# MLAB-project/radio-observer

Measured on AMD Instinct MI355X. Metric: FFT rows/sec (spectra/sec), N=32768 75% overlap, incl. per-row bolid scan, higher is better.
Workload: dtype f32; 1 GPU; C3/C4: synthetic IQ 48 kHz, FFT bins=32768, overlap=24576 (75%), Nuttall window, waterfall magnitude rows + BolidRecorder scan; input=float32 I/Q resident in HBM, output=float32 rows in HBM, parallelism=time-chunk per GPU

## Files before the change

radio-observer_amd/csrc/ro_k32_lds.h:

```cpp
#pragma once

#include "ro_fft_device.h"
#include "ro_device_util.h"

namespace ro {
namespace k32 {

constexpr int N = 32768, T = 1024, H = 16;
constexpr int RQ = 1026;
constexpr int IMAGE_BYTES = 32 * RQ * 4;
constexpr int LDS_BYTES = IMAGE_BYTES + 1024;
constexpr int HB = 61692;
constexpr int XB = 3972;
static_assert(HB % 4 == 0 && 15 * 256 + HB <= 65535 && 31 * 4 * RQ - HB <= 65535 && 16 * 4 * RQ - HB >= 0,
              "rows 16..31: M0 / offset split");
static_assert(XB % 4 == 0 && 15 * 4 * RQ + XB <= 65535 && 4 * 16 * RQ + 15 * 256 - XB <= 65535 && 4 * 16 * RQ - XB >= 0,
              "exchange 1, odd slots: M0 / offset split");

template <int Q>
__device__ __forceinline__ void x1_write_pair(unsigned ma, unsigned mb, float s_q, float s_q1, float s_q16, float s_q17)
{
    static_assert(Q % 2 == 0 && Q < 16, "slot algebra");
    constexpr int E = 256 * (Q >> 1), O = 4 * 16 * RQ - XB + 256 * (Q >> 1);
    addtid_write4<E, E + 2048, O, O + 2048>(ma, mb, s_q, s_q16, s_q1, s_q17);
}
template <typename F> __device__ __forceinline__ void x1_write_plane(unsigned ma, unsigned mb, F f)
{
    constexpr int O = 4 * 16 * RQ - XB;
    addtid_write8<0, 256, 512, 768, 1024, 1280, 1536, 1792>(ma, f(0), f(2), f(4), f(6), f(8), f(10), f(12), f(14));
    addtid_write8<2048, 2304, 2560, 2816, 3072, 3328, 3584, 3840>(ma, f(16), f(18), f(20), f(22), f(24), f(26), f(28), f(30));
    addtid_write8<O, O + 256, O + 512, O + 768, O + 1024, O + 1280, O + 1536, O + 1792>(mb, f(1), f(3), f(5), f(7), f(9), f(11),
                                                                                        f(13), f(15));
    addtid_write8<O + 2048, O + 2304, O + 2560, O + 2816, O + 3072, O + 3328, O + 3584, O + 3840>(
        mb, f(17), f(19), f(21), f(23), f(25), f(27), f(29), f(31));
}
template <int QA, int QB, int QC, int QD>
__device__ __forceinline__ void own_write4(unsigned mc, unsigned md, float sa, float sb, float sc, float sd)
{
    static_assert(QA < 16 && QB < 16 && QC >= 16 && QD >= 16 && QC < 32 && QD < 32, "row algebra");
    constexpr int R = 4 * RQ;
    addtid_write4<R * QA, R * QB, R * QC - HB, R * QD - HB>(mc, md, sa, sb, sc, sd);
}
template <typename F> __device__ __forceinline__ void own_write_plane(unsigned mc, unsigned md, F f)
{
    constexpr int R = 4 * RQ;
    addtid_write8<0 * R, 1 * R, 2 * R, 3 * R, 4 * R, 5 * R, 6 * R, 7 * R>(mc, f(0), f(1), f(2), f(3), f(4), f(5), f(6), f(7));
    addtid_write8<8 * R, 9 * R, 10 * R, 11 * R, 12 * R, 13 * R, 14 * R, 15 * R>(mc, f(8), f(9), f(10), f(11), f(12), f(13),
                                                                                  f(14), f(15));
    addtid_write8<16 * R - HB, 17 * R - HB, 18 * R - HB, 19 * R - HB, 20 * R - HB, 21 * R - HB, 22 * R - HB, 23 * R - HB>(
        md, f(16), f(17), f(18), f(19), f(20), f(21), f(22), f(23));
    addtid_write8<24 * R - HB, 25 * R - HB, 26 * R - HB, 27 * R - HB, 28 * R - HB, 29 * R - HB, 30 * R - HB, 31 * R - HB>(
        md, f(24), f(25), f(26), f(27), f(28), f(29), f(30), f(31));
}

typedef const volatile __attribute__((address_space(3))) v2f lds_vpair;

}
}
```

radio-observer_amd/csrc/ro_stft32k.hip:

```cpp
#define RO_TIE_SCHED 1
#include "ro_kernels.h"
#include "ro_fft_device.h"
#include "ro_fft_planar.h"
#include "ro_device_util.h"
#include "ro_k32_lds.h"

#include <mutex>

#if !defined(RO_DIAG) || !defined(RO_STAMPS32K)
#undef RO_STAMPS32K
#define RO_STAMPS32K 0
#endif

namespace ro {
namespace k32 {

constexpr int PIPE_UNITS = 6;
constexpr int WIN_EARLY = 2;

__host__ __device__ constexpr int column(int t)
{
    const int l = t & 63, j = l & 31;
    return (t & ~63) + 2 * ((j >> 1) + 16 * (j & 1)) + (l >> 5);
}

struct ImageRow {
    const float *img;
    __device__ __forceinline__ float operator()(int c) const
    {
        const int k = (c + N / 2) & (N - 1), r = k >> 10, beta = k & 1023;
        const int w = (beta & 31) >> 1, kb = beta & 1, k1 = beta >> 5;
        return img[RQ * r + 64 * w + 2 * ((k1 - 4 * (w >> 1)) & 31) + kb];
    }
};

template <typename F> __device__ __forceinline__ void dit32_levels123(v2f *v, F hook)
{
    const v2f *tok = &v[31];
    dit_level_order<1>(v, tok, std::make_integer_sequence<int, 2>{});
    hook(std::integral_constant<int, 1>{});
    dit_level_order<2>(v, tok, std::make_integer_sequence<int, 4>{});
    hook(std::integral_constant<int, 2>{});
    dit_level_order<3>(v, tok, std::make_integer_sequence<int, 8>{});
    hook(std::integral_constant<int, 3>{});
}

template <int FMT> __global__ __launch_bounds__(T, 1) void stft32k_kernel(StftArgs a)
{
    extern __shared__ __attribute__((aligned(16))) char smem[];
    using S = Sample<FMT>;
    using namespace planar;

    const int64_t per_xcd = (a.rows + 7) / 8;
    const int64_t xcd_first = (int64_t)(blockIdx.x & 7) * per_xcd;
    const int64_t xcd_end = xcd_first + per_xcd < a.rows ? xcd_first + per_xcd : a.rows;
    const int64_t stride = gridDim.x >> 3;
    int64_t row = xcd_first + (blockIdx.x >> 3);
    if (row >= xcd_end) return;

    const int tid = threadIdx.x;
    const int wave = __builtin_amdgcn_readfirstlane(tid >> 6);
    const __amdgpu_buffer_rsrc_t rs_twk = make_rsrc(a.twiddles_k, (3 * 32 + 3 * 1024) * 16);
    const char *iq = reinterpret_cast<const char *>(a.iq);
    const float *lds = reinterpret_cast<const float *>(smem);

    v2f v[32];

    const int po = (column(tid & ~32) + ((tid >> 5) & 1) * H * (N / 32)) * S::BYTES;
    auto row_rsrc = [&](int64_t k, bool valid) {
        return make_rsrc(iq + (a.first_row + k) * (int64_t)a.hop * S::BYTES, valid ? (unsigned)N * S::BYTES : 0u);
    };
    {
        const __amdgpu_buffer_rsrc_t rs = row_rsrc(row, true);
#pragma unroll
        for (int k = 0; k < H; ++k) S::load_pair(rs, po, k * (N / 32) * S::BYTES, v[k], v[H + k]);
    }
    v4f w4[H / 2];
    auto load_window = [&](const __amdgpu_buffer_rsrc_t &rs_win, auto first_c, auto last_c) {
        constexpr int first = decltype(first_c)::value, last = decltype(last_c)::value;
#pragma unroll
        for (int q = first; q < last; ++q) {
            const u32x4 t = __builtin_amdgcn_raw_buffer_load_b128(rs_win, tid * 16, q * T * 16, 0);
            w4[q] = (v4f){__uint_as_float(t.x), __uint_as_float(t.y), __uint_as_float(t.z), __uint_as_float(t.w)};
        }
    };
    using c0 = std::integral_constant<int, 0>;
    using cE = std::integral_constant<int, WIN_EARLY>;
    using cN = std::integral_constant<int, H / 2>;
    auto win_rsrc = [&](bool valid) { return make_rsrc(a.window_k32, valid ? N * 4 : 0); };
    load_window(win_rsrc(true), c0{}, cN{});

    v2f tw1[5], tw2[5];
    auto tw_load = [&](v2f (&t)[5], int k, auto pk_c, auto ns_c) {
        constexpr int PK = decltype(pk_c)::value, NS = decltype(ns_c)::value;
#pragma unroll
        for (int q = 0; q < 3; ++q) {
            const u32x4 u = __builtin_amdgcn_raw_buffer_load_b128(rs_twk, k * 16, (PK + q * NS) * 16, 0);
            t[2 * q] = (v2f){__uint_as_float(u.x), __uint_as_float(u.y)};
            if (q < 2) t[2 * q + 1] = (v2f){__uint_as_float(u.z), __uint_as_float(u.w)};
        }
    };

    [[maybe_unused]] unsigned long long st_acc[16] = {0, 0, 0, 0, 0, 0, 0, 0, 0, 0, 0, 0, 0, 0, 0, 0}, st_prev = 0;
    auto stamp = [&](int k) {
        if constexpr (RO_STAMPS32K) {
            unsigned long long t;
            __builtin_amdgcn_sched_barrier(0);
            asm volatile("s_memtime %0\n\ts_waitcnt lgkmcnt(0)" : "=s"(t)::"memory");
            __builtin_amdgcn_sched_barrier(0);
            if (k >= 0) st_acc[k] += t - st_prev;
            st_prev = t;
        }
    };
    stamp(-1);
    if constexpr (RO_STAMPS32K) st_acc[13] = __builtin_amdgcn_s_memrealtime();

    const float *prev_out = a.rows_out;
    unsigned prev_bytes = 0;
    unsigned touch = 0;
    int rb_base = RQ * (tid >> 8) + 128 * (tid & 7) + 2 * ((((tid & 255) >> 3) - 4 * (tid & 7)) & 31);
    auto store_chunk = [&](int q, const __amdgpu_buffer_rsrc_t &rs) {
        int rb = rb_base;
        asm volatile("" : "+v"(rb));
        lds_vpair *p = (lds_vpair *)(lds + rb + 4 * RQ * q);
        const v2f x01 = p[0], x23 = p[32];
        buf_store_f4(x01.x, x01.y, x23.x, x23.y, rs, tid * 16, ((q * T * 4 + N / 2) & (N - 1)) * 4);
    };

    const unsigned ma = (unsigned)wave * (4u * RQ), mb = ma + (unsigned)XB;
    const unsigned mc = (unsigned)wave * 256u, md = mc + (unsigned)HB;

    for (;;) {
        const __amdgpu_buffer_rsrc_t rs_prev = make_rsrc(prev_out, prev_bytes);
        {
            const v2f gain2 = (v2f){0.0f, a.gain};
            if (a.gain != 0.0f) {
#pragma unroll
                for (int i = 0; i < 32; ++i) v[i] = v[i] + gain2;
            }
#pragma unroll
            for (int k = 0; k < H; ++k) {
                v2f &lo = v[k], &hi = v[H + k];
                const auto rx = __builtin_amdgcn_permlane32_swap(__float_as_uint(lo.x), __float_as_uint(hi.x), false, false);
                const auto ry = __builtin_amdgcn_permlane32_swap(__float_as_uint(lo.y), __float_as_uint(hi.y), false, false);
                lo = (v2f){__uint_as_float(rx[0]), __uint_as_float(ry[0])};
                hi = (v2f){__uint_as_float(rx[1]), __uint_as_float(ry[1])};
            }
        }
        asm volatile("" ::"v"(touch));
#pragma unroll
        for (int i = 0; i < H; ++i) {
            const v4f c4 = w4[i / 2];
            const v2f wi = (i & 1) ? c4.zz : c4.xx, wj = (i & 1) ? c4.ww : c4.yy;
            const v2f t = v[i] * wi;
            const v2f s = __builtin_elementwise_fma(v[H + i], wj, t);
            v[H + i] = __builtin_elementwise_fma(v[H + i], -wj, t);
            v[i] = s;
            if (i & 1) planar::leash();
        }
        const int64_t next = row + stride;
        const bool has_next = next < xcd_end;
        load_window(win_rsrc(true), c0{}, cE{});
        auto touch_next = [&]() {
            const int64_t s0 = (a.first_row + (has_next ? next : row)) * (int64_t)a.hop + (N - a.hop);
            const __amdgpu_buffer_rsrc_t rs_new =
                make_rsrc(iq + s0 * S::BYTES, (has_next && a.prefetch) ? a.hop * S::BYTES : 0);
            touch = __builtin_amdgcn_raw_buffer_load_b32(rs_new, tid * 128, 0, 0);
        };
        stamp(0);

        store_chunk(0, rs_prev);
        store_chunk(1, rs_prev);
        dit32_levels123(v, [&](auto hc) {
            constexpr int h = decltype(hc)::value;
            store_chunk(2 * h, rs_prev);
            store_chunk(2 * h + 1, rs_prev);
        });
        int lane;
        {
            int lt = tid;
            asm volatile("" : "+v"(lt));
            lane = lt & 63;
        }
        {
            const bool odd = lane >= 32;
            const float4 *tk = a.twiddles_k + 2 * wave;
#pragma unroll
            for (int q = 0; q < 3; ++q) {
                v4f e, o;
                asm volatile("s_load_dwordx4 %0, %2, %3\n\t"
                             "s_load_dwordx4 %1, %2, %4\n\t"
                             "s_waitcnt lgkmcnt(0)"
                             : "=&s"(e), "=&s"(o)
                             : "s"(tk), "n"(q * 32 * 16), "n"(q * 32 * 16 + 16)
                             : "memory");
                tw1[2 * q] = (v2f){odd ? o.x : e.x, odd ? o.y : e.y};
                if (q < 2) tw1[2 * q + 1] = (v2f){odd ? o.z : e.z, odd ? o.w : e.w};
            }
        }
        stamp(1);
        wg_sync();
        stamp(2);
        dit32_last(v, [&](auto jc) {
            constexpr int j = decltype(jc)::value;
            x1_write_pair<bitrev<32>(2 * j)>(ma, mb, v[2 * j].x, v[16 + 2 * j].x, v[2 * j + 1].x, v[17 + 2 * j].x);
            return v[17 + 2 * j].y;
        });
        stamp(3);
        v2f R[16], I[16];
        {
            lds_vpair *g1 = (lds_vpair *)(lds + RQ * 16 * (lane >> 5) + 64 * wave + 2 * (lane & 15) + 32 * ((lane >> 4) & 1));
            asm volatile("s_waitcnt lgkmcnt(0)" ::: "memory");
            __builtin_amdgcn_s_barrier();
            asm volatile("" ::: "memory");
#pragma unroll
            for (int i = 0; i < 16; ++i) R[i] = g1[(RQ / 2) * i];
            wg_sync();
            x1_write_plane(ma, mb, [&](int k0) { return v[bitrev<32>(k0)].y; });
            asm volatile("s_waitcnt lgkmcnt(0)" ::: "memory");
            __builtin_amdgcn_s_barrier();
            asm volatile("" ::: "memory");
#pragma unroll
            for (int i = 0; i < 8; ++i) {
                I[i] = g1[(RQ / 2) * i];
                I[i + 8] = g1[(RQ / 2) * (i + 8)];
            }
        }
        stamp(4);
        planar::head<0>(R, I, tw1[4], tw1[3], tw1[2], tw1[1]);
        touch_next();
        int k1p, kbp;
        {
            k1p = ((lane >> 1) + 4 * (wave >> 1)) & 31;
            kbp = lane & 1;
            tw_load(tw2, 2 * wave + kbp + 32 * k1p, std::integral_constant<int, 96>{}, std::integral_constant<int, 1024>{});
        }
        stamp(5);
        planar::last0(R, I, tw1[0], [&](auto jc) {
            constexpr int j = decltype(jc)::value, q = bitrev<32>(2 * j);
            own_write4<q, q + 1, q + 16, q + 17>(mc, md, R[j].x, R[8 + j].x, R[j].y, R[8 + j].y);
        });
        stamp(6);
        v2f R2[16], I2[16];
        {
            lds_vpair *g2 = (lds_vpair *)(lds + RQ * k1p + 64 * wave + 32 * kbp);
            asm volatile("" ::: "memory");
#pragma unroll
            for (int i = 0; i < 16; ++i) R2[i] = g2[(i >> 1) + 8 * (i & 1)];
            asm volatile("" ::: "memory");
            own_write_plane(mc, md, [&](int k1) {
                constexpr int MB = 0;
                const int p = bitrev<32>(k1);
                return hf<MB>(p) ? I[pr<MB>(p)].y : I[pr<MB>(p)].x;
            });
#pragma unroll
            for (int i = 0; i < 16; ++i) I2[i] = g2[(i >> 1) + 8 * (i & 1)];
        }
        stamp(7);
        planar::head<1>(R2, I2, tw2[4], tw2[3], tw2[2], tw2[1]);
        stamp(8);
        {
            const __amdgpu_buffer_rsrc_t rs_next = row_rsrc(has_next ? next : row, has_next);
            v2f pma = {0.f, 0.f}, pmb = {0.f, 0.f};
            planar::last1(R2, I2, tw2[0], [&](auto uc) {
                constexpr int u = decltype(uc)::value;
                auto mag = [](v2f re, v2f im) {
                    const v2f s = __builtin_elementwise_fma(im, im, re * re);
                    return (v2f){__builtin_amdgcn_sqrtf(s.x), __builtin_amdgcn_sqrtf(s.y)};
                };
                const v2f m_a = mag(R2[2 * u], I2[2 * u]), m_b = mag(R2[2 * u + 1], I2[2 * u + 1]);
                if constexpr (u > 0) {
                    constexpr int r = bitrev<8>(u > 0 ? u - 1 : 0);
                    own_write4<r, r + 8, r + 16, r + 24>(mc, md, pma.x, pma.y, pmb.x, pmb.y);
                }
                pma = m_a;
                pmb = m_b;
                if constexpr (u < PIPE_UNITS) {
                    const int pj = after(po, m_b.y);
                    S::load_pair(rs_next, pj, (2 * u) * (N / 32) * S::BYTES, v[2 * u], v[H + 2 * u]);
                    S::load_pair(rs_next, pj, (2 * u + 1) * (N / 32) * S::BYTES, v[2 * u + 1], v[H + 2 * u + 1]);
                }
            });
            asm volatile("s_nop 7\n\ts_nop 7" ::: "memory");
            {
                constexpr int r = bitrev<8>(7);
                own_write4<r, r + 8, r + 16, r + 24>(mc, md, pma.x, pma.y, pmb.x, pmb.y);
            }
            const bool image_work = (a.records != nullptr && wave < 2) || (a.tile_out != nullptr && (wave == 2 || wave == 3));
            auto late_loads = [&]() {
#pragma unroll
                for (int k = 2 * PIPE_UNITS; k < H; ++k)
                    S::load_pair(rs_next, po, k * (N / 32) * S::BYTES, v[k], v[H + k]);
                load_window(win_rsrc(has_next), cE{}, cN{});
            };
            auto image_complete = [&]() {
                stamp(9);
                asm volatile("s_waitcnt lgkmcnt(0)" ::: "memory");
                wg_sync();
                stamp(10);
            };
            if (!image_work) {
                late_loads();
                image_complete();
            } else {
                image_complete();
                {
                    int sl = tid & 63;
                    asm volatile("" : "+v"(sl));
                    const ImageRow img{lds};
                    if (a.records != nullptr && wave < 2) {
                        int low_noise = a.low_noise, noise_width = a.noise_width, low_detect = a.low_detect;
                        int detect_width = a.detect_width, avg_bins = a.avg_bins;
                        asm volatile("" : "+s"(low_noise), "+s"(noise_width), "+s"(low_detect), "+s"(detect_width), "+s"(avg_bins));
                        if (wave == 0) {
                            unsigned *hist = reinterpret_cast<unsigned *>(smem + IMAGE_BYTES);
                            const float nz = noise_width <= 512 ? scan_noise<8>(img, low_noise, noise_width, hist, sl)
                                                                : scan_noise<0>(img, low_noise, noise_width, hist, sl);
                            if (sl == 0) a.records[row].noise = nz;
                        } else {
                            const int pk = scan_peak<8>(img, low_detect, detect_width, sl);
                            const float av = scan_average(img, low_detect + pk - avg_bins / 2, avg_bins, N, sl);
                            if (sl == 0) {
                                a.records[row].peak = pk;
                                a.records[row].average = av;
                            }
                        }
                    }
                    if (a.tile_out != nullptr && (wave == 2 || wave == 3)) {
                        int tile_cols = a.tile_cols, tile_first = a.tile_first;
                        asm volatile("" : "+s"(tile_cols), "+s"(tile_first));
                        const int half = ((tile_cols + 127) >> 7) << 6;
                        const int c0 = wave == 2 ? 0 : half;
                        const int c1 = wave == 2 ? (half < tile_cols ? half : tile_cols) : tile_cols;
                        float *dst = a.tile_out + row * (int64_t)tile_cols;
                        if (a.ln_out == nullptr) {
                            for (int c = c0 + sl; c < c1; c += 64) dst[c] = img(tile_first + c);
                        } else {
                            float *ldst = a.ln_out + row * (int64_t)tile_cols;
                            unsigned kmin = 0xffffffffu, kmax = 0u;
                            for (int c = c0 + sl; c < c1; c += 64) {
                                const float x = img(tile_first + c);
                                const float l = logf(x);
                                dst[c] = x;
                                ldst[c] = l;
                                if (x != 0.f) {
                                    const unsigned key = order_key(l);
                                    kmin = min(kmin, key);
                                    kmax = max(kmax, key);
                                }
                            }
                            kmin = wave_min_u32(kmin);
                            kmax = wave_max_u32(kmax);
                            if (sl == 0) {
                                float *part = a.ln_part + row * 4 + (wave == 2 ? 0 : 2);
                                part[0] = kmin == 0xffffffffu ? __builtin_inff() : key_to_float(kmin);
                                part[1] = kmax == 0u ? -__builtin_inff() : key_to_float(kmax);
                            }
                        }
                    }
                }
                late_loads();
            }
        }
        stamp(11);
        prev_out = a.rows_out + row * a.row_stride;
        prev_bytes = N * 4;
        if constexpr (RO_STAMPS32K) st_acc[15] += 1;
        if (!has_next) break;
        row = next;
    }
    {
        const __amdgpu_buffer_rsrc_t rs_last = make_rsrc(prev_out, prev_bytes);
#pragma unroll
        for (int q = 0; q < 8; ++q) {
            store_chunk(q, rs_last);
            if (q & 1) asm volatile("" ::: "memory");
        }
    }
    if constexpr (RO_STAMPS32K) {
        st_acc[14] = __builtin_amdgcn_s_memrealtime();
        if (a.stamps && (tid & 63) == 0)
            for (int k = 0; k < 16; ++k) a.stamps[(blockIdx.x * 16 + wave) * 16 + k] = st_acc[k];
    }
}

struct DevicePlan32k {
    bool ready = false;
    int cus = 0;
};

template <int FMT> static hipError_t launch_fmt(const StftArgs &a, hipStream_t s)
{
    static std::mutex lock;
    static DevicePlan32k table[64];
    int dev = 0;
    hipError_t e = hipGetDevice(&dev);
    if (e != hipSuccess) return e;
    if (dev < 0 || dev >= 64) return hipErrorInvalidDevice;
    int cus;
    {
        std::lock_guard<std::mutex> g(lock);
        DevicePlan32k &d = table[dev];
        if (!d.ready) {
            const void *fn = reinterpret_cast<const void *>(&stft32k_kernel<FMT>);
            if ((e = hipFuncSetAttribute(fn, hipFuncAttributeMaxDynamicSharedMemorySize, LDS_BYTES)) != hipSuccess) return e;
            if ((e = hipDeviceGetAttribute(&d.cus, hipDeviceAttributeMultiprocessorCount, dev)) != hipSuccess) return e;
            d.ready = true;
        }
        cus = d.cus;
    }
    const int64_t per_xcd = (a.rows + 7) / 8;
    int64_t slots = cus / 8;
    if (a.spare_cus > 0) slots -= a.spare_cus;
    if (slots < 1) slots = 1;
    if (slots > per_xcd) slots = per_xcd;
    StftArgs b = a;
    b.dec = 1;
    b.dec_log2 = 0;
    b.prefetch = slots * (int64_t)a.hop * Sample<FMT>::BYTES <= (2 << 20) ? 1 : 0;
    b.stagger = 0;
    hipLaunchKernelGGL((stft32k_kernel<FMT>), dim3((unsigned)(slots * 8)), dim3(T), LDS_BYTES, s, b);
    return hipGetLastError();
}

}

void stft32k_window_layout(const float *w, float *out)
{
    using namespace k32;
    for (int t = 0; t < T; ++t) {
        const int c = column(t);
        for (int q = 0; q < H / 2; ++q) {
            float *o = out + ((size_t)q * T + t) * 4;
            o[0] = w[c + 1024 * (2 * q)];
            o[1] = w[c + 1024 * (2 * q + 16)];
            o[2] = w[c + 1024 * (2 * q + 1)];
            o[3] = w[c + 1024 * (2 * q + 17)];
        }
    }
}

hipError_t launch_stft32k(int fmt, const StftArgs &a, hipStream_t s)
{
    if (a.rows <= 0) return hipSuccess;
    if (a.spec_out != nullptr || a.big_form || a.window_k32 == nullptr) return hipErrorInvalidValue;
    if (fmt == RO_FMT_F32) return k32::launch_fmt<RO_FMT_F32>(a, s);
    if (fmt == RO_FMT_I16) return k32::launch_fmt<RO_FMT_I16>(a, s);
    return hipErrorInvalidValue;
}

}
```

Before: 17.56 million rows/s.

## Reschedule first LDS exchange with parked young-wave values and split twiddle loads

New measurement: 16.89 million rows/s. 0.962x the previous value.

```diff
diff --git a/radio-observer_amd/csrc/ro_k32_lds.h b/radio-observer_amd/csrc/ro_k32_lds.h
--- a/radio-observer_amd/csrc/ro_k32_lds.h
+++ b/radio-observer_amd/csrc/ro_k32_lds.h
@@ -17,22 +17,28 @@
 static_assert(XB % 4 == 0 && 15 * 4 * RQ + XB <= 65535 && 4 * 16 * RQ + 15 * 256 - XB <= 65535 && 4 * 16 * RQ - XB >= 0,
               "exchange 1, odd slots: M0 / offset split");
 
+__host__ __device__ constexpr int x1_offset(int k0) { return 256 * (k0 >> 1) + (k0 & 1) * (4 * 16 * RQ - XB); }
+__host__ __device__ constexpr int x1_park_offset(int k0) { return x1_offset(k0 - 16); }
+static_assert(x1_park_offset(16) == 0 && x1_park_offset(17) == 4 * 16 * RQ - XB && x1_park_offset(31) == x1_offset(15),
+              "phase 1 parks y of slot k0 in territory (k0 >> 1) - 8");
+static_assert(x1_park_offset(16) >= 0 && x1_park_offset(31) <= 65535 && x1_park_offset(30) + 15 * 4 * RQ + 252 < IMAGE_BYTES &&
+                  x1_park_offset(31) + 15 * 4 * RQ + XB + 252 < IMAGE_BYTES,
+              "exchange 1, parked y values: M0 / offset split, inside the image");
+static_assert(x1_park_offset(30) + 256 <= x1_offset(16), "parked y values stay below territory 8");
+
 template <int Q>
-__device__ __forceinline__ void x1_write_pair(unsigned ma, unsigned mb, float s_q, float s_q1, float s_q16, float s_q17)
+__device__ __forceinline__ void x1_write_young(unsigned ma, unsigned mb, float x_q16, float y_q16, float x_q17, float y_q17)
 {
     static_assert(Q % 2 == 0 && Q < 16, "slot algebra");
-    constexpr int E = 256 * (Q >> 1), O = 4 * 16 * RQ - XB + 256 * (Q >> 1);
-    addtid_write4<E, E + 2048, O, O + 2048>(ma, mb, s_q, s_q16, s_q1, s_q17);
+    addtid_write4<x1_park_offset(Q + 16), x1_offset(Q + 16), x1_park_offset(Q + 17), x1_offset(Q + 17)>(ma, mb, y_q16, x_q16,
+                                                                                                      y_q17, x_q17);
 }
-template <typename F> __device__ __forceinline__ void x1_write_plane(unsigned ma, unsigned mb, F f)
+template <typename F> __device__ __forceinline__ void x1_write_old(unsigned ma, unsigned mb, F f)
 {
-    constexpr int O = 4 * 16 * RQ - XB;
+    constexpr int O = x1_offset(1);
     addtid_write8<0, 256, 512, 768, 1024, 1280, 1536, 1792>(ma, f(0), f(2), f(4), f(6), f(8), f(10), f(12), f(14));
-    addtid_write8<2048, 2304, 2560, 2816, 3072, 3328, 3584, 3840>(ma, f(16), f(18), f(20), f(22), f(24), f(26), f(28), f(30));
     addtid_write8<O, O + 256, O + 512, O + 768, O + 1024, O + 1280, O + 1536, O + 1792>(mb, f(1), f(3), f(5), f(7), f(9), f(11),
                                                                                         f(13), f(15));
-    addtid_write8<O + 2048, O + 2304, O + 2560, O + 2816, O + 3072, O + 3328, O + 3584, O + 3840>(
-        mb, f(17), f(19), f(21), f(23), f(25), f(27), f(29), f(31));
 }
 template <int QA, int QB, int QC, int QD>
 __device__ __forceinline__ void own_write4(unsigned mc, unsigned md, float sa, float sb, float sc, float sd)
diff --git a/radio-observer_amd/csrc/ro_stft32k.hip b/radio-observer_amd/csrc/ro_stft32k.hip
--- a/radio-observer_amd/csrc/ro_stft32k.hip
+++ b/radio-observer_amd/csrc/ro_stft32k.hip
@@ -160,7 +160,6 @@
         }
         const int64_t next = row + stride;
         const bool has_next = next < xcd_end;
-        load_window(win_rsrc(true), c0{}, cE{});
         auto touch_next = [&]() {
             const int64_t s0 = (a.first_row + (has_next ? next : row)) * (int64_t)a.hop + (N - a.hop);
             const __amdgpu_buffer_rsrc_t rs_new =
@@ -182,11 +181,11 @@
             asm volatile("" : "+v"(lt));
             lane = lt & 63;
         }
-        {
+        auto load_tw1 = [&](auto first_c, auto last_c) {
             const bool odd = lane >= 32;
             const float4 *tk = a.twiddles_k + 2 * wave;
 #pragma unroll
-            for (int q = 0; q < 3; ++q) {
+            for (int q = decltype(first_c)::value; q < decltype(last_c)::value; ++q) {
                 v4f e, o;
                 asm volatile("s_load_dwordx4 %0, %2, %3\n\t"
                              "s_load_dwordx4 %1, %2, %4\n\t"
@@ -197,37 +196,76 @@
                 tw1[2 * q] = (v2f){odd ? o.x : e.x, odd ? o.y : e.y};
                 if (q < 2) tw1[2 * q + 1] = (v2f){odd ? o.z : e.z, odd ? o.w : e.w};
             }
-        }
+        };
         stamp(1);
         wg_sync();
         stamp(2);
+        const bool young = wave >= 8;
         dit32_last(v, [&](auto jc) {
             constexpr int j = decltype(jc)::value;
-            x1_write_pair<bitrev<32>(2 * j)>(ma, mb, v[2 * j].x, v[16 + 2 * j].x, v[2 * j + 1].x, v[17 + 2 * j].x);
+            x1_write_young<bitrev<32>(2 * j)>(ma, mb, v[2 * j + 1].x, v[2 * j + 1].y, v[17 + 2 * j].x, v[17 + 2 * j].y);
             return v[17 + 2 * j].y;
         });
         stamp(3);
         v2f R[16], I[16];
+        using cH = std::integral_constant<int, 4>;
+        using cQ = std::integral_constant<int, 8>;
+        auto pass1_level0_a = [&]() {
+            const v2f lvl0[8] = {tw1[4]};
+            planar::bf_all<0, 0>(R, I, lvl0, std::integer_sequence<int, 0, 2, 4, 6>{});
+        };
+        auto pass1_level0_b = [&]() {
+            const v2f lvl0[8] = {tw1[4]};
+            planar::bf_all<0, 0>(R, I, lvl0, std::integer_sequence<int, 8, 10, 12, 14>{});
+        };
+        auto not_yet = [&](v2f (&P)[16], auto first_c, auto last_c) {
+#pragma unroll
+            for (int i = decltype(first_c)::value; i < decltype(last_c)::value; ++i) asm volatile("" : "=v"(P[i]), "=v"(P[i + 8]));
+        };
         {
             lds_vpair *g1 = (lds_vpair *)(lds + RQ * 16 * (lane >> 5) + 64 * wave + 2 * (lane & 15) + 32 * ((lane >> 4) & 1));
+            auto read_plane = [&](v2f (&P)[16], lds_vpair *g, auto first_c, auto last_c) {
+#pragma unroll
+                for (int i = decltype(first_c)::value; i < decltype(last_c)::value; ++i) {
+                    P[i] = g[(RQ / 2) * i];
+                    P[i + 8] = g[(RQ / 2) * (i + 8)];
+                }
+            };
             asm volatile("s_waitcnt lgkmcnt(0)" ::: "memory");
             __builtin_amdgcn_s_barrier();
             asm volatile("" ::: "memory");
-#pragma unroll
-            for (int i = 0; i < 16; ++i) R[i] = g1[(RQ / 2) * i];
+            if (young) read_plane(I, g1 - 64 * 8 / 2, c0{}, cQ{});
+            else not_yet(I, c0{}, cQ{});
             wg_sync();
-            x1_write_plane(ma, mb, [&](int k0) { return v[bitrev<32>(k0)].y; });
+            stamp(4);
+            x1_write_old(ma, mb, [&](int k0) { return v[bitrev<32>(k0)].x; });
+            if (young) read_plane(R, g1, c0{}, cH{});
+            else not_yet(R, c0{}, cH{});
+            not_yet(R, cH{}, cQ{});
+            load_tw1(std::integral_constant<int, 2>{}, std::integral_constant<int, 3>{});
             asm volatile("s_waitcnt lgkmcnt(0)" ::: "memory");
             __builtin_amdgcn_s_barrier();
             asm volatile("" ::: "memory");
-#pragma unroll
-            for (int i = 0; i < 8; ++i) {
-                I[i] = g1[(RQ / 2) * i];
-                I[i + 8] = g1[(RQ / 2) * (i + 8)];
-            }
-        }
-        stamp(4);
-        planar::head<0>(R, I, tw1[4], tw1[3], tw1[2], tw1[1]);
+            if (young) pass1_level0_a();
+            else read_plane(R, g1, c0{}, cQ{});
+            wg_sync();
+            x1_write_old(ma, mb, [&](int k0) { return v[bitrev<32>(k0)].y; });
+            if (young) read_plane(R, g1, cH{}, cQ{});
+            load_tw1(c0{}, std::integral_constant<int, 2>{});
+            asm volatile("s_waitcnt lgkmcnt(0)" ::: "memory");
+            __builtin_amdgcn_s_barrier();
+            asm volatile("" ::: "memory");
+            if (!young) {
+                read_plane(I, g1, c0{}, cQ{});
+                pass1_level0_a();
+            }
+            pass1_level0_b();
+        }
+        stamp(12);
+        load_window(win_rsrc(true), c0{}, cE{});
+        planar::level<0, 1>(R, I, tw1[3]);
+        planar::level<0, 2>(R, I, tw1[2]);
+        planar::level<0, 3>(R, I, tw1[1]);
         touch_next();
         int k1p, kbp;
         {
```
